# basilevh/occlusions-4d

Hardware: AMD Instinct MI355X
Metric: 4D query-points/sec (encode+decode) at n_points=14336 (higher is better)
Workload: dtype f32; 1 GPU; GREATER inference (BASELINE configs[1]): n_points=14336 video_len=12 num_sample=524288 (-> 534528 grid queries) implicit_batch_size=32768 (decoded in mini-batches of 32256 = 3584 workgroups of 9 queries; every query is decoded, results do not depend on the split), seeded random-init weights; abstract_points=531, outputs_per_query=5, parallelism=single GPU, schedule=sequential, rccl_ranks=1, decode_streams=2, decode_chunk=32256

## Files before the change

occlusions-4d_amd/csrc/common.hpp:

```cpp
#pragma once
#include <hip/hip_runtime.h>
#include <stdint.h>
#include <stdio.h>

#include "contract.hpp"

namespace occ4d {

inline int check_launch(const char* what) {
  hipError_t e = hipGetLastError();
  if (e != hipSuccess) {
    set_error("%s: %s", what, hipGetErrorString(e));
    return OCC4D_ELAUNCH;
  }
  return OCC4D_OK;
}

inline int cdiv(int64_t a, int64_t b) { return (int)((a + b - 1) / b); }

template <class Args>
int check_trunk_args(const Args& a, const char* who, int width) {
  OCC4D_REQUIRE(a.x && a.y && a.w0p && a.b0, "%s: null pointer", who);
  OCC4D_REQUIRE(a.n >= 0, "%s: n = %d", who, a.n);
  OCC4D_REQUIRE(a.ldx >= width && a.ldx % 4 == 0 && a.ldy % 4 == 0 && ((uintptr_t)a.x % 16) == 0 &&
// ... 14 lines not shown
                n_out, stage);
  const bool res_ok = a.ldr % 4 == 0 && ((uintptr_t)a.res % 16) == 0 && a.ldr >= n_out;
  if (skip) {
    OCC4D_REQUIRE(a.res && res_ok, "%s: skip rows must be 16-byte aligned with lds %% 4 == 0 and lds >= n_out", who);
  } else {
    OCC4D_REQUIRE(!a.res || res_ok, "%s: residual rows must be 16-byte aligned with ldr %% 4 == 0", who);
  }
  OCC4D_REQUIRE(!masked || (a.mask && a.ldm % 4 == 0 && ((uintptr_t)a.mask % 16) == 0 && a.ldm >= n_out),
                "%s: mask rows must be 16-byte aligned with ldm %% 4 == 0 and ldm >= n_out", who);
  return OCC4D_OK;
}

constexpr int FPS_BUCKET_MIN_POINTS = 1536;
int fps_bucket_launch(const float* xyz, int64_t stride, int n, int m, int start, int32_t* out_sorted,
                      int32_t* out_order, hipStream_t stream);


bool wgrad16_plan(int M, int N, int K, int* splits, int* m_per_split);
int wgrad16_launch(const float* g, int64_t ldg, const float* x, int64_t ldx, int M, int N, int K, int splits,
                   int m_per_split, float* part, float* part_b, int relu_x, hipStream_t stream);

int zero_rows(float* dst, int64_t ld, int64_t n, int d, hipStream_t st);
int copy_rows(float* dst, int64_t ldd, const float* src, int64_t lds, int64_t n, int d, hipStream_t st);

int cu_count();

bool f16w_enabled();
bool f16_resblock_enabled();

int pack_rowlin_f16x3_prescaled(const float* w, int64_t ldw, int n_out, float prescale, float* packed, hipStream_t st);
int rowlin_f16x3_prescaled(const float* x, int64_t ldx, float* y, int64_t ldy, const float* w_packed, const float* b,
                           int n_out, float prescale, int relu_in, const float* res, int64_t ldr, int n, hipStream_t st);

int attn16p_skew();

}
```

occlusions-4d_amd/csrc/path.hip:

```cpp
#include <algorithm>
#include <stdio.h>
#include <stdlib.h>

#include "common.hpp"

namespace {

using occ4d::cdiv;

#define TRY(expr)                  \
  do {                             \
    const int rc_ = (expr);        \
    if (rc_ != OCC4D_OK) return rc_; \
  } while (0)

constexpr int TRUNK = 416;
constexpr int ROW_CHUNK = 32768;
inline int row_step(int n) {
  static const bool balance = [] { const char* e = getenv("OCC4D_ROW_BALANCE"); return !e || e[0] != '0'; }();
  const int passes = (n + ROW_CHUNK - 1) / ROW_CHUNK;
  return passes <= 1 || !balance ? ROW_CHUNK : ((n + passes - 1) / passes + 8) / 9 * 9;
}
constexpr int64_t ALIGN = 64;

// ... 323 lines not shown
      snprintf(what, sizeof(what), "%s, merged query projection W1 Wq", who);
      TRY(check_f16_stream(prep + L.wq_x6, split_packed_floats(true, 2 * D), flag, what, "packed stream", st));
      snprintf(what, sizeof(what), "%s, layer3 weight", who);
      TRY(check_f16_stream(prep + L.w3_x6, split_packed_floats(true, w.d_out), flag, what, "packed stream", st));
    }
    if (L.bf16x6) {
      snprintf(what, sizeof(what), "%s, attention weights (attn_mlp[2] W2, merged Wp = W1 P2, pos_mlp[2] P2)", who);
      TRY(check_f16_stream(prep + L.stream6, L.f16w ? occ4d_pt_cross_attn_f16w_stream_floats()
                                                    : occ4d_pt_cross_attn_f16x3_stream_floats(), flag, what, "packed stream", st));
    }
  }
  return OCC4D_OK;
}

struct SceneTables { int64_t kt, vt, vtc, total; };
SceneTables scene_layout(const occ4d_pt_layer_weights& w, int m) {
  SceneTables s{};
  s.kt = 0;
  s.vt = up((int64_t)m * 2 * w.dim);
  s.vtc = s.vt + up((int64_t)m * w.dim);
  s.total = s.vtc + up((int64_t)m * w.dim);
  return s;
}
int layer_scene(const occ4d_pt_layer_weights& w, const LayerLayout& L, const float* prep, const float* x2, int64_t ldx2,
                int m, float* scene, hipStream_t st) {
  const SceneTables s = scene_layout(w, m);
  const int D = L.D, D2 = L.D2;
  TRY(lin(x2, ldx2, prep + L.wk, D2, nullptr, scene + s.kt, 2 * D, m, D2, 2 * D, 0, 0, nullptr, 0, st));
  TRY(lin(x2, ldx2, w.to_v, D2, nullptr, scene + s.vt, D, m, D2, D, 0, 0, nullptr, 0, st));
  TRY(lin(x2, ldx2, w.to_v, D2, w.pos2_b, scene + s.vtc, D, m, D2, D, 0, 0, nullptr, 0, st));
  return OCC4D_OK;
}

int rowlin_any(bool trunk4, const float* x, int64_t ldx, float* y, int64_t ldy, const float* wpk, const float* b, int n_out,
               int relu_in, const float* res, int64_t ldr, int n, const Events& E, hipStream_t st) {
  E.before(OCC4D_PROFILE_ROWLIN);
  const int rc = trunk4
      ? occ4d_rowlin4_f32(x, ldx, y, ldy, wpk, b, n_out, relu_in, res, ldr, nullptr, nullptr, 0, nullptr, nullptr, 0, n, st)
      : occ4d_rowlin_f32(x, ldx, y, ldy, wpk, b, n_out, relu_in, res, ldr, nullptr, nullptr, 0, nullptr, nullptr, 0, n, st);
  E.after(OCC4D_PROFILE_ROWLIN);
  return rc;
}

int rowlin_x6(bool f16, const float* x, int64_t ldx, float* y, int64_t ldy, const float* wpk, const float* b, int n_out,
              int relu_in, const float* res, int64_t ldr, int n, const Events& E, hipStream_t st, float prescale = 1.f) {
  E.before(OCC4D_PROFILE_ROWLIN);
  const int rc = split_rowlin(f16, x, ldx, y, ldy, wpk, b, n_out, relu_in, res, ldr, n, st, prescale);
  E.after(OCC4D_PROFILE_ROWLIN);
  return rc;
}

int layer_forward(const occ4d_pt_layer_weights& w, const LayerLayout& L, const float* prep, const float* x, int64_t ldx,
                  const float* pos, int64_t ps, int n, const float* x2, int64_t ldx2, const float* pos2, int64_t p2s, int m,
                  int k, const int32_t* knn_idx, const float* scene, float* out, int64_t ldo, Bump& ws,
                  const Events& E, hipStream_t st, bool dry, float* logits_out = nullptr, float* a_out = nullptr,
                  float* pe_out = nullptr) {
  const int D = L.D, h = L.h;
  const int64_t mark = ws.mark();
  const float *kt, *vt, *vtc, *aq_all = nullptr, *yfeat = x;
  int64_t ld_y = ldx;
  if (!w.cross) {
    if (w.pre_w) {
      float* y = ws.take((int64_t)n * D);
      if (!dry) TRY(lin(x, ldx, w.pre_w, w.d_in, w.pre_b, y, D, n, w.d_in, D, 0, 0, nullptr, 0, st));
      yfeat = y; ld_y = D;
    }
    float* ktb = ws.take((int64_t)n * 2 * D);
    float* vtb = ws.take((int64_t)n * D);
    float* vcb = (L.fused16p || L.bf16x6) ? ws.take((int64_t)n * D) : nullptr;
    float* aqb = ws.take((int64_t)n * 2 * D);
    if (!dry) {
      TRY(lin(yfeat, ld_y, prep + L.wk, D, nullptr, ktb, 2 * D, n, D, 2 * D, 0, 0, nullptr, 0, st));
      TRY(lin(yfeat, ld_y, w.to_v, D, nullptr, vtb, D, n, D, D, 0, 0, nullptr, 0, st));
      if (vcb) TRY(lin(yfeat, ld_y, w.to_v, D, w.pos2_b, vcb, D, n, D, D, 0, 0, nullptr, 0, st));
      TRY(lin(yfeat, ld_y, prep + L.wq, D, prep + L.bq, aqb, 2 * D, n, D, 2 * D, 0, 0, nullptr, 0, st));
    }
    kt = ktb; vt = vtb; vtc = vcb; aq_all = aqb;
    pos2 = pos; p2s = ps; m = n;
  } else if (scene) {
    const SceneTables s = scene_layout(w, m);
    kt = scene + s.kt; vt = scene + s.vt; vtc = scene + s.vtc;
  } else {
    const SceneTables s = scene_layout(w, m);
    float* tb = ws.take(s.total);
    if (!dry) TRY(layer_scene(w, L, prep, x2, ldx2, m, tb, st));
    kt = tb + s.kt; vt = tb + s.vt; vtc = tb + s.vtc;
  }
  float* agg = out;
  int64_t ld_agg = ldo;
// ... 68 lines not shown
          rc = occ4d_pt_cross_attn_f32(aq, 2 * D, qp, ps, pos2, p2s, idx, kt, 2 * D, vt, D, w.pos0_w, w.pos0_b, prep + L.wp,
                                       w.attn2_w, w.attn2_b, w.pos2_w, w.pos2_b, agg_c, ld_agg, c, m, k, D, divisor, st);
        E.after(OCC4D_PROFILE_CROSS_ATTN);
        TRY(rc);
      }
    } else if (L.fused_self16 && k == 16) {
      if (!dry)
        TRY(occ4d_pt_self_attn16_f32(aq, 2 * D, qp, ps, pos2, p2s, idx, kt, 2 * D, vt, D, w.pos0_w, w.pos0_b, prep + L.wp,
                                     w.attn2_w, w.pos2_w, w.pos2_b, agg_c, ld_agg, c, m, k, D, divisor, st));
    } else {
      const int64_t rows = (int64_t)c * k;
      float* r = ws.take(rows * h);
      float* hid = ws.take(rows * 2 * D);
      float* logits = ws.take(rows * D);
      float* pe = ws.take(rows * D);
      if (!dry) {
        TRY(occ4d_pt_pos_hidden_f32(qp, ps, pos2, p2s, idx, c, k, w.pos0_w, w.pos0_b, h, r, st));
        occ4d_linear_args a{};
        a.x = r; a.ldx = h; a.w = prep + L.wp; a.ldw = h; a.y = hid; a.ldy = 2 * D;
        a.M = (int)rows; a.K = h; a.N = 2 * D; a.relu_out = 1;
        a.add_rows = aq; a.ld_add = 2 * D; a.add_div = k; a.sub_rows = kt; a.ld_sub = 2 * D; a.sub_idx = idx;
        TRY(occ4d_linear_f32(&a, st));
        TRY(lin(hid, 2 * D, w.attn2_w, 2 * D, w.attn2_b, logits, D, (int)rows, 2 * D, D, 0, 0, nullptr, 0, st));
        TRY(lin(r, h, w.pos2_w, h, w.pos2_b, pe, D, (int)rows, h, D, 0, 0, nullptr, 0, st));
        TRY(occ4d_pt_softmax_agg_f32(logits, vt, D, pe, idx, c, k, D, divisor, agg_c, ld_agg, st));
      }
    }
    ws.release(cmark);
  }
  if (w.post_w && !dry) {
    if (L.x6rows)
      TRY(rowlin_x6(L.f16, agg, D, out, ldo, prep + L.w3_x6, w.post_b, w.d_out, 0, x, ldx, n, E, st));
    else if (L.w3_rows)
      TRY(rowlin_any(L.trunk4, agg, D, out, ldo, prep + L.w3_packed, w.post_b, w.d_out, 0, x, ldx, n, E, st));
    else
      TRY(lin(agg, D, w.post_w, D, w.post_b, out, ldo, n, D, w.d_out, 0, 0, x, ldx, st));
  }
  ws.release(mark);
  return OCC4D_OK;
}

struct DecoderLayout {
  int H, P, P4, dg, E, nB, nC;
  bool trunk, trunk4, resblock;
  bool x6trunk;
  bool f16;
  bool f16block;
  int64_t w0p[OCC4D_MAX_BLOCKS], w1p[OCC4D_MAX_BLOCKS];
  int64_t w0x[OCC4D_MAX_BLOCKS], w1x[OCC4D_MAX_BLOCKS];
  int64_t cross[OCC4D_MAX_CROSS];
  LayerLayout cl[OCC4D_MAX_CROSS];
  int64_t total;
};

int check_decoder(const occ4d_decoder_weights* w, const char* who) {
  OCC4D_REQUIRE(w, "%s: null weights", who);
  OCC4D_REQUIRE(w->n_blocks >= 1 && w->n_blocks <= OCC4D_MAX_BLOCKS && w->n_cross >= 0 && w->n_cross <= OCC4D_MAX_CROSS,
                "%s: n_blocks = %d (1 .. %d), n_cross = %d (0 .. %d)", who, w->n_blocks, OCC4D_MAX_BLOCKS, w->n_cross,
                OCC4D_MAX_CROSS);
  OCC4D_REQUIRE(w->d_hidden % 4 == 0 && w->d_hidden >= 4 && w->d_out >= 1 && w->d_in >= 3 && w->n_freq >= 0,
                "%s: d_hidden = %d must be a multiple of 4, d_in = %d >= 3 (x, y, z first)", who, w->d_hidden, w->d_in);
  const int P = w->d_in * (2 * w->n_freq + 1);
  OCC4D_REQUIRE(w->lin_in_ld >= P && w->lin_in_ld % 4 == 0, "%s: lin_in_ld = %d must be a multiple of 4 >= %d (zero-pad "
                "lin_in.weight's rows)", who, w->lin_in_ld, P);
  OCC4D_REQUIRE(w->d_latent_local >= 4 && w->d_latent_local % 4 == 0 && w->d_latent >= w->d_latent_local &&
                    (w->d_latent - w->d_latent_local) % 4 == 0,
                "%s: d_latent = %d, d_latent_local = %d (both parts multiples of 4; local_mode 'feature' / 'attention')",
// ... 84 lines not shown
    const int64_t mark = ws.mark();
    const float* q = queries + (int64_t)lo * qs;
    float* x = penult ? penult + (int64_t)lo * ld_pen : ws.take((int64_t)c * H);
    const int64_t ldx = penult ? ld_pen : H;
    int32_t* idx8 = reinterpret_cast<int32_t*>(ws.take((int64_t)c * w.k_local));
    float* w8 = ws.take((int64_t)c * w.k_local);
    int32_t* idx_att = L.nC ? reinterpret_cast<int32_t*>(ws.take((int64_t)c * w.k_cross)) : nullptr;
    float* pe = ws.take((int64_t)c * L.P4);
    float* hbuf = (L.resblock && (!L.x6trunk || L.f16block)) ? nullptr : ws.take((int64_t)c * H);
    if (!dry) {
      if (knn_local) {
        TRY(clamp_indices(knn_local + (int64_t)lo * w.k_local, (int64_t)c * w.k_local, m, idx8, st));
        TRY(occ4d_knn_dists_f32(q, qs, c, xyz, 3, m, idx8, w.k_local, 1, w8, st));
      } else {
        TRY(occ4d_knn_f32(q, qs, c, xyz, 3, m, w.k_local, 1, idx8, 0, w8, st));
      }
      TRY(occ4d_interp_weights_f32(w8, c, w.k_local, w8, st));
      if (L.nC && knn_cross) TRY(clamp_indices(knn_cross + (int64_t)lo * w.k_cross, (int64_t)c * w.k_cross, m, idx_att, st));
      else if (L.nC) TRY(occ4d_knn_f32(q, qs, c, xyz, 3, m, w.k_cross, 0, idx_att, 0, nullptr, st));
      const float* emb = q;
      int64_t ld_emb = qs;
      if (w.n_freq > 0) {
        if (L.P4 != L.P) TRY(occ4d::zero_rows(pe, L.P4, c, L.P4, st));
        TRY(occ4d_posenc_f32(q, qs, c, w.d_in, w.n_freq, (double)w.base_frequency, pe, L.P4, st));
        emb = pe; ld_emb = L.P4;
      } else {
        TRY(occ4d::zero_rows(pe, L.P4, c, L.P4, st));
        TRY(occ4d::copy_rows(pe, L.P4, q, qs, c, w.d_in, st));
        emb = pe; ld_emb = L.P4;
      }
      TRY(lin(emb, ld_emb, w.lin_in_w, w.lin_in_ld, w.lin_in_b, x, ldx, c, L.P4, H, 0, 0, nullptr, 0, st));
    }
    int next_cross = 0;
    for (int i = 0; i < L.nB; ++i) {
      if (!dry) {
        const bool fuse_ok = (flags & OCC4D_PATH_FUSED_INTERP) && L.resblock && !L.trunk4;
        const bool cross_behind = next_cross < L.nC && w.cross_after[next_cross] == i;
        const bool cross_before = i > 0 && next_cross > 0 && w.cross_after[next_cross - 1] == i - 1;
        const bool had_it = fuse_ok && i > 0 && !cross_before;
        const bool give_next = fuse_ok && i + 1 < L.nB && !cross_behind;
        if (!had_it)
          TRY(occ4d_interp_add_f32(x, ldx, scene + S.zconst + (int64_t)i * H, scene + S.ztab + (int64_t)i * H,
                                   (int64_t)L.nB * H, idx8, w8, c, w.k_local, H, st));
        if (L.f16block) {
          E.before(OCC4D_PROFILE_RESBLOCK);
          const int rc = occ4d_resblock_f16x3_f32(x, ldx, x, ldx, prep + L.w0x[i], w.fc0_b[i], w.fc1_b[i], c, st);
          E.after(OCC4D_PROFILE_RESBLOCK);
          TRY(rc);
        } else if (L.x6trunk) {
          E.before(OCC4D_PROFILE_RESBLOCK);
          int rc = split_rowlin(L.f16, x, ldx, hbuf, H, prep + L.w0x[i], w.fc0_b[i], H, 1, nullptr, 0, c, st);
          if (!rc) rc = split_rowlin(L.f16, hbuf, H, x, ldx, prep + L.w1x[i], w.fc1_b[i], H, 1, x, ldx, c, st);
          E.after(OCC4D_PROFILE_RESBLOCK);
          TRY(rc);
        } else if (L.resblock) {
          E.before(OCC4D_PROFILE_RESBLOCK);
          const float* zc = give_next ? scene + S.zconst + (int64_t)(i + 1) * H : nullptr;
          const float* zt = give_next ? scene + S.ztab + (int64_t)(i + 1) * H : nullptr;
          const int rc = L.trunk4
              ? occ4d_resblock4_f32(x, ldx, x, ldx, prep + L.w0p[i], w.fc0_b[i], prep + L.w1p[i], w.fc1_b[i], nullptr,
                                    nullptr, 0, nullptr, nullptr, 0, c, st)
              : occ4d_resblock_f32(x, ldx, x, ldx, prep + L.w0p[i], w.fc0_b[i], prep + L.w1p[i], w.fc1_b[i], zc, zt,
                                   (int64_t)L.nB * H, give_next ? idx8 : nullptr, give_next ? w8 : nullptr,
                                   give_next ? w.k_local : 0, c, st);
          E.after(OCC4D_PROFILE_RESBLOCK);
          TRY(rc);
        } else {
          TRY(lin(x, ldx, w.fc0_w[i], H, w.fc0_b[i], hbuf, H, c, H, H, act, 0, nullptr, 0, st));
          TRY(lin(hbuf, H, w.fc1_w[i], H, w.fc1_b[i], x, ldx, c, H, H, act, 0, x, ldx, st));
        }
      }
      if (next_cross < L.nC && w.cross_after[next_cross] == i) {
        const int j = next_cross++;
        TRY(layer_forward(w.cross[j], L.cl[j], prep ? prep + L.cross[j] : nullptr, x, ldx, q, qs, c, nullptr, 0, xyz, 3, m,
                          w.k_cross, idx_att, scene ? scene + S.layer[j] : nullptr, x, ldx, ws, E, st, dry));
      }
    }
    if (!dry)
      TRY(lin(x, ldx, w.lin_out_w, H, w.lin_out_b, out + (int64_t)lo * ld_out, ld_out, c, H, w.d_out, act, 0, nullptr, 0, st));
    ws.release(mark);
  }
  (void)flags;
  return OCC4D_OK;
}

}

namespace occ4d {
bool f16_resblock_enabled() {
  static const bool v = [] {
    const char* e = getenv("OCC4D_F16_RESBLOCK");
    return !e || atoi(e) != 0;
  }();
  return v;
}
bool f16w_enabled() {
  static const bool v = [] {
    const char* e = getenv("OCC4D_F16W");
    return e && atoi(e) != 0;
  }();
  return v;
}
int attn16p_skew() {
  static const int v = [] {
    const char* e = getenv("OCC4D_CA16P_SKEW");
    return e ? atoi(e) : 6;
  }();
  return v;
}
}

extern "C" int occ4d_pack_trunk_rows_f32(const float* w, int64_t ldw, int n_out, float* packed, void* stream) {
  OCC4D_REQUIRE(w && packed && n_out >= 32 && n_out % 32 == 0 && ldw >= TRUNK,
                "occ4d_pack_trunk_rows_f32: (%d, %d) weight with n_out %% 32 == 0 expected", n_out, TRUNK);
  const int64_t total = occ4d_trunk_packed_floats(n_out);
  pack_trunk_rows_kernel<<<cdiv(total, 256), 256, 0, (hipStream_t)stream>>>(w, ldw, n_out / 32, packed);
  return occ4d::check_launch("occ4d_pack_trunk_rows_f32");
}
extern "C" int occ4d_pack_trunk_cols_f32(const float* w, int64_t ldw, float* packed, void* stream) {
  OCC4D_REQUIRE(w && packed && ldw >= TRUNK, "occ4d_pack_trunk_cols_f32: (416, 416) weight expected");
  pack_trunk_cols_kernel<<<cdiv((int64_t)14 * 13312, 256), 256, 0, (hipStream_t)stream>>>(w, ldw, packed);
  return occ4d::check_launch("occ4d_pack_trunk_cols_f32");
}
extern "C" int occ4d_pack_trunk4_rows_f32(const float* w, int64_t ldw, int n_out, float* packed, void* stream) {
  OCC4D_REQUIRE(w && packed && n_out >= 16 && n_out % 16 == 0 && ldw >= TRUNK,
// ... 234 lines not shown
```

occlusions-4d_amd/csrc/trunk.hip:

```cpp
#include "tile.hpp"

namespace {

constexpr int TH = 416;
constexpr int TKG = TH / 16;
constexpr int TNS = TH / 32;
constexpr int FRAG_FLOATS = 256;
constexpr int STAGE_FRAGS = 2 * TKG;
constexpr int STAGE_FLOATS = STAGE_FRAGS * FRAG_FLOATS;
constexpr int TROWS = 128;

struct TrunkArgs {
  const float* x; int64_t ldx;
  float* y; int64_t ldy;
  const float* w0p; const float* b0;
  const float* w1p; const float* b1;
  const float* res; int64_t ldr;
  const float* zconst; const float* ztab; int64_t ldz; const int32_t* zidx; const float* zw; int kz;
  int n;
  int n_stages;
  int relu_in;
  const float* mask; int64_t ldm;
};

__device__ __forceinline__ void dma_stage(const float* __restrict__ src, const float* dst, int wave, int lane) {
#pragma unroll
  for (int i = 0; i < 7; ++i) {
    const int c = wave + 8 * i;
    if (c < STAGE_FRAGS) dma_frag(src + c * FRAG_FLOATS, lds_addr(dst) + (unsigned)c * (FRAG_FLOATS * 4), (unsigned)lane * 16u);
  }
}

__device__ __forceinline__ void dma_part(const float* __restrict__ src, const float* dst, int wave, int lane, int i) {
  const int c = wave + 8 * i;
  if (c < STAGE_FRAGS) dma_frag(src + c * FRAG_FLOATS, lds_addr(dst) + (unsigned)c * (FRAG_FLOATS * 4), (unsigned)lane * 16u);
}

__device__ __forceinline__ void interp_into(const TrunkArgs& a, int rowc, int g, f32x4* out) {
#pragma unroll
  for (int t = 0; t < TKG; ++t) {
    const f32x4 c = *reinterpret_cast<const f32x4*>(a.zconst + 16 * t + 4 * g);
    out[t].x += c.x; out[t].y += c.y; out[t].z += c.z; out[t].w += c.w;
  }
  for (int j = 0; j < a.kz; ++j) {
    const float w = a.zw[(int64_t)rowc * a.kz + j];
    const float* zr = a.ztab + (int64_t)a.zidx[(int64_t)rowc * a.kz + j] * a.ldz + 4 * g;
#pragma unroll
    for (int t = 0; t < TKG; ++t) {
      const f32x4 z = *reinterpret_cast<const f32x4*>(zr + 16 * t);
      out[t].x = fmaf(w, z.x, out[t].x); out[t].y = fmaf(w, z.y, out[t].y);
      out[t].z = fmaf(w, z.z, out[t].z); out[t].w = fmaf(w, z.w, out[t].w);
    }
  }
}

__global__ __launch_bounds__(512, 2) void resblock_kernel(const TrunkArgs a) {
  __shared__ __attribute__((aligned(16))) float bufA[STAGE_FLOATS];
  __shared__ __attribute__((aligned(16))) float bufB[STAGE_FLOATS];
  __shared__ __attribute__((aligned(16))) float s_b0[TH];
  const int tid = threadIdx.x, lane = tid & 63, wave = __builtin_amdgcn_readfirstlane(tid >> 6);
  const int r = lane & 15, g = lane >> 4;
  const int row = blockIdx.x * TROWS + wave * 16 + r;
  const int rowc = min(row, a.n - 1);

  dma_stage(a.w0p, bufA, wave, lane);
  if (tid < TH) s_b0[tid] = a.b0[tid];
  f32x4 xr[TKG], yacc[TKG];
  {
    const float* xp = a.x + (int64_t)rowc * a.ldx + 4 * g;
#pragma unroll
    for (int t = 0; t < TKG; ++t) {
#ifdef OCC4D_TR_NOPRO
      const f32x4 v = {(float)t, (float)g, (float)r, 1.f};
#else
      const f32x4 v = *reinterpret_cast<const f32x4*>(xp + 16 * t);
#endif
      const f32x4 b = *reinterpret_cast<const f32x4*>(a.b1 + 16 * t + 4 * g);
      xr[t] = relu4(v);
      yacc[t].x = v.x + b.x; yacc[t].y = v.y + b.y; yacc[t].z = v.z + b.z; yacc[t].w = v.w + b.w;
    }
  }
  dma_wait();
  __syncthreads();
  const float* const fa = bufA + lane * 4;
  const float* const fb = bufB + lane * 4;

#ifdef OCC4D_TR_STAMP
  unsigned long long tacc[4] = {0, 0, 0, 0};
  unsigned long long tprev = __builtin_amdgcn_s_memtime();
  const unsigned long long tstart = tprev;
#define STAMP(i) { const unsigned long long tn = __builtin_amdgcn_s_memtime(); tacc[i] += tn - tprev; tprev = tn; }
#else
#define STAMP(i)
#endif
  asm volatile("; OCC4D_MARK loop");
#pragma clang loop unroll(disable)
  for (int j = 0; j < TNS; ++j) {
    f32x4 h0 = *reinterpret_cast<const f32x4*>(s_b0 + 32 * j + 4 * g);
    f32x4 h1 = *reinterpret_cast<const f32x4*>(s_b0 + 32 * j + 16 + 4 * g);
    {
      f32x4 wa = *reinterpret_cast<const f32x4*>(fa);
      f32x4 wb = *reinterpret_cast<const f32x4*>(fa + TKG * FRAG_FLOATS);
#pragma unroll
      for (int t = 0; t < TKG; ++t) {
#ifndef OCC4D_TR_NODMA
        if (t >= 2 && t <= 20 && (t - 2) % 3 == 0) dma_part(a.w1p + (int64_t)j * STAGE_FLOATS, bufB, wave, lane, (t - 2) / 3);
#endif
        const f32x4 ca = wa, cb = wb;
        if (t + 1 < TKG) {
          wa = *reinterpret_cast<const f32x4*>(fa + (t + 1) * FRAG_FLOATS);
          wb = *reinterpret_cast<const f32x4*>(fa + (TKG + t + 1) * FRAG_FLOATS);
        }
        __builtin_amdgcn_sched_barrier(0);
        mfma16x2_b(ca, cb, xr[t], h0, h1);
// ... 12 lines not shown
      f32x4 wa = *reinterpret_cast<const f32x4*>(fb);
      f32x4 wb = *reinterpret_cast<const f32x4*>(fb + 2 * FRAG_FLOATS);
#pragma unroll
      for (int q = 0; q < TKG; ++q) {
        const int p = q >> 1, tt = q & 1;
#ifndef OCC4D_TR_NODMA
        if (q >= 2 && q <= 20 && (q - 2) % 3 == 0) dma_part(a.w0p + (int64_t)(j + 1) * STAGE_FLOATS, bufA, wave, lane, (q - 2) / 3);
#endif
        const f32x4 ca = wa, cb = wb;
        if (q + 1 < TKG) {
          const int pn = (q + 1) >> 1, tn = (q + 1) & 1;
          wa = *reinterpret_cast<const f32x4*>(fb + (4 * pn + tn) * FRAG_FLOATS);
          wb = *reinterpret_cast<const f32x4*>(fb + (4 * pn + 2 + tn) * FRAG_FLOATS);
        }
        __builtin_amdgcn_sched_barrier(0);
        mfma16x2_b(ca, cb, tt ? h1 : h0, yacc[2 * p], yacc[2 * p + 1]);
        __builtin_amdgcn_sched_barrier(0);
      }
    }
    STAMP(2)
#ifndef OCC4D_TR_NOBAR
    dma_wait();
    __syncthreads();
#endif
    STAMP(3)
  }
  asm volatile("; OCC4D_MARK epilogue");
#ifdef OCC4D_TR_STAMP
  if (lane == 0 && a.zw) {
    unsigned long long* o = (unsigned long long*)a.zw + (size_t)(blockIdx.x * 8 + wave) * 6;
    o[0] = tacc[0]; o[1] = tacc[1]; o[2] = tacc[2]; o[3] = tacc[3]; o[4] = tprev - tstart; o[5] = tstart;
  }
#endif
  if (a.ztab) interp_into(a, rowc, g, yacc);
#ifdef OCC4D_TR_NOEPI
  {
    float tsum = 0.f;
#pragma unroll
    for (int t = 0; t < TKG; ++t) tsum += yacc[t].x + yacc[t].y + yacc[t].z + yacc[t].w;
    if (tsum == 123.456f) a.y[0] = tsum;
    return;
  }
#endif
  if (row < a.n) {
    float* yp = a.y + (int64_t)row * a.ldy + 4 * g;
#pragma unroll
    for (int t = 0; t < TKG; ++t) *reinterpret_cast<f32x4*>(yp + 16 * t) = yacc[t];
  }
}

__device__ __forceinline__ void rowlin_stage(const TrunkArgs& a, int s, const float* __restrict__ frag, const f32x4* xr,
                                             int row, int rowc, int g, const float* next_src, const float* next_dst,
                                             int wave, int lane) {
  const int c0 = 32 * s + 4 * g;
  const f32x4 bz0 = *reinterpret_cast<const f32x4*>(a.b0 + c0);
  const f32x4 bz1 = *reinterpret_cast<const f32x4*>(a.b0 + c0 + 16);
  f32x4 o0 = {0.f, 0.f, 0.f, 0.f}, o1 = {0.f, 0.f, 0.f, 0.f};
  f32x4 r0 = {0.f, 0.f, 0.f, 0.f}, r1 = {0.f, 0.f, 0.f, 0.f};
  if (a.res) {
    r0 = *reinterpret_cast<const f32x4*>(a.res + (int64_t)rowc * a.ldr + c0);
    r1 = *reinterpret_cast<const f32x4*>(a.res + (int64_t)rowc * a.ldr + c0 + 16);
  }
  {
    f32x4 wa = *reinterpret_cast<const f32x4*>(frag);
    f32x4 wb = *reinterpret_cast<const f32x4*>(frag + TKG * FRAG_FLOATS);
#pragma unroll
    for (int t = 0; t < TKG; ++t) {
      if (t >= 2 && t <= 20 && (t - 2) % 3 == 0) dma_part(next_src, next_dst, wave, lane, (t - 2) / 3);
      const f32x4 ca = wa, cb = wb;
      if (t + 1 < TKG) {
        wa = *reinterpret_cast<const f32x4*>(frag + (t + 1) * FRAG_FLOATS);
        wb = *reinterpret_cast<const f32x4*>(frag + (TKG + t + 1) * FRAG_FLOATS);
      }
      __builtin_amdgcn_sched_barrier(0);
      mfma16x2_b(ca, cb, xr[t], o0, o1);
      __builtin_amdgcn_sched_barrier(0);
    }
  }
  o0.x += bz0.x + r0.x; o0.y += bz0.y + r0.y; o0.z += bz0.z + r0.z; o0.w += bz0.w + r0.w;
  o1.x += bz1.x + r1.x; o1.y += bz1.y + r1.y; o1.z += bz1.z + r1.z; o1.w += bz1.w + r1.w;
  if (a.ztab) {
    const f32x4 ca = *reinterpret_cast<const f32x4*>(a.zconst + c0);
    const f32x4 cb = *reinterpret_cast<const f32x4*>(a.zconst + c0 + 16);
    o0.x += ca.x; o0.y += ca.y; o0.z += ca.z; o0.w += ca.w;
    o1.x += cb.x; o1.y += cb.y; o1.z += cb.z; o1.w += cb.w;
    for (int j = 0; j < a.kz; ++j) {
      const float w = a.zw[(int64_t)rowc * a.kz + j];
      const float* zr = a.ztab + (int64_t)a.zidx[(int64_t)rowc * a.kz + j] * a.ldz + c0;
      const f32x4 za = *reinterpret_cast<const f32x4*>(zr);
      const f32x4 zb = *reinterpret_cast<const f32x4*>(zr + 16);
      o0.x = fmaf(w, za.x, o0.x); o0.y = fmaf(w, za.y, o0.y); o0.z = fmaf(w, za.z, o0.z); o0.w = fmaf(w, za.w, o0.w);
      o1.x = fmaf(w, zb.x, o1.x); o1.y = fmaf(w, zb.y, o1.y); o1.z = fmaf(w, zb.z, o1.z); o1.w = fmaf(w, zb.w, o1.w);
    }
  }
  if (a.mask) {
    const f32x4 m0 = *reinterpret_cast<const f32x4*>(a.mask + (int64_t)rowc * a.ldm + c0);
    const f32x4 m1 = *reinterpret_cast<const f32x4*>(a.mask + (int64_t)rowc * a.ldm + c0 + 16);
    o0.x = m0.x > 0.f ? o0.x : 0.f; o0.y = m0.y > 0.f ? o0.y : 0.f; o0.z = m0.z > 0.f ? o0.z : 0.f; o0.w = m0.w > 0.f ? o0.w : 0.f;
    o1.x = m1.x > 0.f ? o1.x : 0.f; o1.y = m1.y > 0.f ? o1.y : 0.f; o1.z = m1.z > 0.f ? o1.z : 0.f; o1.w = m1.w > 0.f ? o1.w : 0.f;
  }
  if (row < a.n) {
    float* yp = a.y + (int64_t)row * a.ldy + c0;
    *reinterpret_cast<f32x4*>(yp) = o0;
    *reinterpret_cast<f32x4*>(yp + 16) = o1;
  }
}

__global__ __launch_bounds__(512, 2) void rowlin_kernel(const TrunkArgs a) {
  __shared__ __attribute__((aligned(16))) float bufA[STAGE_FLOATS];
  __shared__ __attribute__((aligned(16))) float bufB[STAGE_FLOATS];
  const int tid = threadIdx.x, lane = tid & 63, wave = __builtin_amdgcn_readfirstlane(tid >> 6);
  const int r = lane & 15, g = lane >> 4;
  const int row = blockIdx.x * TROWS + wave * 16 + r;
  const int rowc = min(row, a.n - 1);
  dma_stage(a.w0p, bufA, wave, lane);
  f32x4 xr[TKG];
  {
    const float* xp = a.x + (int64_t)rowc * a.ldx + 4 * g;
#pragma unroll
    for (int t = 0; t < TKG; ++t) {
      const f32x4 v = *reinterpret_cast<const f32x4*>(xp + 16 * t);
      xr[t] = a.relu_in ? relu4(v) : v;
    }
  }
  dma_wait();
  __syncthreads();
#pragma clang loop unroll(disable)
  for (int s = 0; s < a.n_stages; s += 2) {
    rowlin_stage(a, s, bufA + lane * 4, xr, row, rowc, g, a.w0p + (int64_t)(s + 1) * STAGE_FLOATS, bufB, wave, lane);
    dma_wait();
    __syncthreads();
    if (s + 1 < a.n_stages)
      rowlin_stage(a, s + 1, bufB + lane * 4, xr, row, rowc, g, a.w0p + (int64_t)(s + 2) * STAGE_FLOATS, bufA, wave, lane);
    dma_wait();
    __syncthreads();
  }
}

int rowlin_launch(const char* who, const float* x, int64_t ldx, float* y, int64_t ldy, const float* w_packed, const float* b,
                  int n_out, int relu_in, const float* res, int64_t ldr, const float* zconst, const float* ztab, int64_t ldz,
                  const int32_t* zidx, const float* zw, int kz, bool masked, const float* mask, int64_t ldm, int n,
                  void* stream) {
  if (n == 0) return OCC4D_OK;
  TrunkArgs a{x, ldx, y, ldy, w_packed, b, nullptr, nullptr, res, ldr, zconst, ztab, ldz, zidx, zw, kz, n,
              n_out / 32, relu_in, mask, ldm};
  if (int rc = occ4d::check_rowlin_args(a, who, TH, 32, n_out, masked)) return rc;
  rowlin_kernel<<<occ4d::cdiv(n, TROWS), 512, 0, (hipStream_t)stream>>>(a);
  return occ4d::check_launch(who);
}

}

extern "C" int occ4d_trunk_width(void) { return TH; }
extern "C" int64_t occ4d_trunk_packed_floats(int n_out) { return (int64_t)(n_out / 32 + 1) * STAGE_FLOATS; }

extern "C" int occ4d_resblock_f32(const float* x, int64_t ldx, float* y, int64_t ldy, const float* w0_packed,
                                  const float* b0, const float* w1_packed, const float* b1, const float* zconst,
                                  const float* ztab, int64_t ldz, const int32_t* zidx, const float* zw, int kz, int n,
                                  void* stream) {
  TrunkArgs a{x, ldx, y, ldy, w0_packed, b0, w1_packed, b1, nullptr, 0, zconst, ztab, ldz, zidx, zw, kz, n, TNS, 1, nullptr, 0};
  if (n == 0) return OCC4D_OK;
  if (int rc = occ4d::check_trunk_args(a, "occ4d_resblock_f32", TH)) return rc;
  OCC4D_REQUIRE(w1_packed && b1 && ((uintptr_t)w1_packed % 16) == 0 && ((uintptr_t)b1 % 16) == 0 && ldy >= TH,
                "occ4d_resblock_f32: second layer weights / bias missing or misaligned");
  resblock_kernel<<<occ4d::cdiv(n, TROWS), 512, 0, (hipStream_t)stream>>>(a);
  return occ4d::check_launch("occ4d_resblock_f32");
// ... 17 lines not shown
```

Baseline: 4.529 million query-points/s.

## Stage deduplicated interpolation rows in LDS and fuse interp into cross-layer rowlin

Each 128-row workgroup deduplicates its kNN indices into a small LDS row table using a bitmap, prefix sums and slot indices. The distinct z-table rows are staged into shared memory, reusing the freed stage buffers in resblock and a double-buffered slice image in rowlin. Interpolation then gathers from LDS instead of scattered global loads, and falls back to direct gathers when a tile has more than 64 distinct rows. Separately, the path fuses the next block's interpolation term into the cross-attention output rowlin, removing a standalone interp_add launch. The costs are extra LDS and barriers, which may reduce occupancy, plus the dedupe overhead.

```diff
diff --git a/occlusions-4d_amd/csrc/common.hpp b/occlusions-4d_amd/csrc/common.hpp
--- a/occlusions-4d_amd/csrc/common.hpp
+++ b/occlusions-4d_amd/csrc/common.hpp
@@ -70,6 +70,8 @@
 int rowlin_f16x3_prescaled(const float* x, int64_t ldx, float* y, int64_t ldy, const float* w_packed, const float* b,
                            int n_out, float prescale, int relu_in, const float* res, int64_t ldr, int n, hipStream_t st);
 
+bool staged_interp_enabled();
+
 int attn16p_skew();
 
 }
diff --git a/occlusions-4d_amd/csrc/path.hip b/occlusions-4d_amd/csrc/path.hip
--- a/occlusions-4d_amd/csrc/path.hip
+++ b/occlusions-4d_amd/csrc/path.hip
@@ -379,12 +379,15 @@
   return OCC4D_OK;
 }
 
+struct ZTerm { const float* zconst; const float* ztab; int64_t ldz; const int32_t* idx; const float* w; int k; };
+
 int rowlin_any(bool trunk4, const float* x, int64_t ldx, float* y, int64_t ldy, const float* wpk, const float* b, int n_out,
-               int relu_in, const float* res, int64_t ldr, int n, const Events& E, hipStream_t st) {
+               int relu_in, const float* res, int64_t ldr, int n, const Events& E, hipStream_t st, const ZTerm* z = nullptr) {
   E.before(OCC4D_PROFILE_ROWLIN);
   const int rc = trunk4
       ? occ4d_rowlin4_f32(x, ldx, y, ldy, wpk, b, n_out, relu_in, res, ldr, nullptr, nullptr, 0, nullptr, nullptr, 0, n, st)
-      : occ4d_rowlin_f32(x, ldx, y, ldy, wpk, b, n_out, relu_in, res, ldr, nullptr, nullptr, 0, nullptr, nullptr, 0, n, st);
+      : z ? occ4d_rowlin_f32(x, ldx, y, ldy, wpk, b, n_out, relu_in, res, ldr, z->zconst, z->ztab, z->ldz, z->idx, z->w, z->k, n, st)
+          : occ4d_rowlin_f32(x, ldx, y, ldy, wpk, b, n_out, relu_in, res, ldr, nullptr, nullptr, 0, nullptr, nullptr, 0, n, st);
   E.after(OCC4D_PROFILE_ROWLIN);
   return rc;
 }
@@ -401,7 +404,7 @@
                   const float* pos, int64_t ps, int n, const float* x2, int64_t ldx2, const float* pos2, int64_t p2s, int m,
                   int k, const int32_t* knn_idx, const float* scene, float* out, int64_t ldo, Bump& ws,
                   const Events& E, hipStream_t st, bool dry, float* logits_out = nullptr, float* a_out = nullptr,
-                  float* pe_out = nullptr) {
+                  float* pe_out = nullptr, const ZTerm* zterm = nullptr) {
   const int D = L.D, h = L.h;
   const int64_t mark = ws.mark();
   const float *kt, *vt, *vtc, *aq_all = nullptr, *yfeat = x;
@@ -536,7 +539,7 @@
     if (L.x6rows)
       TRY(rowlin_x6(L.f16, agg, D, out, ldo, prep + L.w3_x6, w.post_b, w.d_out, 0, x, ldx, n, E, st));
     else if (L.w3_rows)
-      TRY(rowlin_any(L.trunk4, agg, D, out, ldo, prep + L.w3_packed, w.post_b, w.d_out, 0, x, ldx, n, E, st));
+      TRY(rowlin_any(L.trunk4, agg, D, out, ldo, prep + L.w3_packed, w.post_b, w.d_out, 0, x, ldx, n, E, st, zterm));
     else
       TRY(lin(agg, D, w.post_w, D, w.post_b, out, ldo, n, D, w.d_out, 0, 0, x, ldx, st));
   }
@@ -687,13 +690,15 @@
       TRY(lin(emb, ld_emb, w.lin_in_w, w.lin_in_ld, w.lin_in_b, x, ldx, c, L.P4, H, 0, 0, nullptr, 0, st));
     }
     int next_cross = 0;
+    const bool fuse_cross = L.resblock && !L.trunk4 && !L.x6trunk && occ4d::staged_interp_enabled();
+    const bool fuse_ok = fuse_cross || ((flags & OCC4D_PATH_FUSED_INTERP) && L.resblock && !L.trunk4 && !L.x6trunk);
+    bool had_it = false;
     for (int i = 0; i < L.nB; ++i) {
+      const bool cross_behind = next_cross < L.nC && w.cross_after[next_cross] == i;
+      const bool give_next = fuse_ok && i + 1 < L.nB && !cross_behind;
+      const bool cross_gives = !dry && fuse_cross && i + 1 < L.nB && cross_behind && L.cl[next_cross].w3_rows &&
+                               !L.cl[next_cross].x6rows && !L.cl[next_cross].trunk4 && w.cross[next_cross].d_out == H;
       if (!dry) {
-        const bool fuse_ok = (flags & OCC4D_PATH_FUSED_INTERP) && L.resblock && !L.trunk4;
-        const bool cross_behind = next_cross < L.nC && w.cross_after[next_cross] == i;
-        const bool cross_before = i > 0 && next_cross > 0 && w.cross_after[next_cross - 1] == i - 1;
-        const bool had_it = fuse_ok && i > 0 && !cross_before;
-        const bool give_next = fuse_ok && i + 1 < L.nB && !cross_behind;
         if (!had_it)
           TRY(occ4d_interp_add_f32(x, ldx, scene + S.zconst + (int64_t)i * H, scene + S.ztab + (int64_t)i * H,
                                    (int64_t)L.nB * H, idx8, w8, c, w.k_local, H, st));
@@ -725,11 +730,17 @@
           TRY(lin(hbuf, H, w.fc1_w[i], H, w.fc1_b[i], x, ldx, c, H, H, act, 0, x, ldx, st));
         }
       }
-      if (next_cross < L.nC && w.cross_after[next_cross] == i) {
+      if (cross_behind) {
         const int j = next_cross++;
+        ZTerm zt{};
+        if (cross_gives)
+          zt = ZTerm{scene + S.zconst + (int64_t)(i + 1) * H, scene + S.ztab + (int64_t)(i + 1) * H, (int64_t)L.nB * H, idx8, w8,
+                     w.k_local};
         TRY(layer_forward(w.cross[j], L.cl[j], prep ? prep + L.cross[j] : nullptr, x, ldx, q, qs, c, nullptr, 0, xyz, 3, m,
-                          w.k_cross, idx_att, scene ? scene + S.layer[j] : nullptr, x, ldx, ws, E, st, dry));
+                          w.k_cross, idx_att, scene ? scene + S.layer[j] : nullptr, x, ldx, ws, E, st, dry, nullptr, nullptr,
+                          nullptr, cross_gives ? &zt : nullptr));
       }
+      had_it = give_next || cross_gives;
     }
     if (!dry)
       TRY(lin(x, ldx, w.lin_out_w, H, w.lin_out_b, out + (int64_t)lo * ld_out, ld_out, c, H, w.d_out, act, 0, nullptr, 0, st));
@@ -746,6 +757,13 @@
   static const bool v = [] {
     const char* e = getenv("OCC4D_F16_RESBLOCK");
     return !e || atoi(e) != 0;
+  }();
+  return v;
+}
+bool staged_interp_enabled() {
+  static const bool v = [] {
+    const char* e = getenv("OCC4D_STAGED_INTERP");
+    return !e || e[0] != '0';
   }();
   return v;
 }
diff --git a/occlusions-4d_amd/csrc/rowstage.hpp b/occlusions-4d_amd/csrc/rowstage.hpp
--- /dev/null
+++ b/occlusions-4d_amd/csrc/rowstage.hpp
@@ -0,0 +1,61 @@
+#pragma once
+#include "common.hpp"
+
+namespace {
+
+constexpr int RS_THREADS = 512;
+constexpr int RS_ROWS = 128;
+constexpr int RS_KMAX = 16;
+constexpr int RS_BITS = 32 * RS_THREADS;
+constexpr int RS_CAP = 64;
+
+struct RowStage {
+  unsigned char slot[RS_ROWS * RS_KMAX];
+  unsigned bm[RS_THREADS];
+  unsigned short pre[RS_THREADS];
+  int rows[RS_CAP];
+  unsigned wsum[RS_THREADS / 64];
+  int bad;
+};
+
+__device__ __forceinline__ int rs_dedupe(RowStage& rs, const int32_t* __restrict__ idx, int nrefs, int tid) {
+  const int lane = tid & 63, wave = tid >> 6;
+  rs.bm[tid] = 0u;
+  if (tid == 0) rs.bad = 0;
+  __syncthreads();
+  for (int e = tid; e < nrefs; e += RS_THREADS) {
+    const int j = idx[e];
+    if ((unsigned)j < (unsigned)RS_BITS) atomicOr(&rs.bm[j >> 5], 1u << (j & 31));
+    else rs.bad = 1;
+  }
+  __syncthreads();
+  const unsigned mine = rs.bm[tid];
+  const unsigned cnt = (unsigned)__builtin_popcount(mine);
+  unsigned inc = cnt;
+#pragma unroll
+  for (int o = 1; o < 64; o <<= 1) {
+    const unsigned v = (unsigned)__shfl_up((int)inc, o, 64);
+    if (lane >= o) inc += v;
+  }
+  if (lane == 63) rs.wsum[wave] = inc;
+  __syncthreads();
+  unsigned below = 0, total = 0;
+#pragma unroll
+  for (int w = 0; w < RS_THREADS / 64; ++w) {
+    const unsigned s = rs.wsum[w];
+    if (w < wave) below += s;
+    total += s;
+  }
+  if (rs.bad || total > (unsigned)RS_CAP) return -1;
+  unsigned at = below + inc - cnt;
+  rs.pre[tid] = (unsigned short)at;
+  for (unsigned b = mine; b; b &= b - 1) rs.rows[at++] = 32 * tid + (__builtin_ffs((int)b) - 1);
+  __syncthreads();
+  for (int e = tid; e < nrefs; e += RS_THREADS) {
+    const int j = idx[e];
+    rs.slot[e] = (unsigned char)(rs.pre[j >> 5] + __builtin_popcount(rs.bm[j >> 5] & ((1u << (j & 31)) - 1u)));
+  }
+  return (int)total;
+}
+
+}
diff --git a/occlusions-4d_amd/csrc/trunk.hip b/occlusions-4d_amd/csrc/trunk.hip
--- a/occlusions-4d_amd/csrc/trunk.hip
+++ b/occlusions-4d_amd/csrc/trunk.hip
@@ -1,4 +1,5 @@
 #include "tile.hpp"
+#include "rowstage.hpp"
 
 namespace {
 
@@ -9,6 +10,7 @@
 constexpr int STAGE_FRAGS = 2 * TKG;
 constexpr int STAGE_FLOATS = STAGE_FRAGS * FRAG_FLOATS;
 constexpr int TROWS = 128;
+static_assert(TROWS == RS_ROWS && RS_CAP * TH <= 2 * STAGE_FLOATS, "the staged interpolation term lives in the two stage buffers");
 
 struct TrunkArgs {
   const float* x; int64_t ldx;
@@ -36,28 +38,72 @@
   if (c < STAGE_FRAGS) dma_frag(src + c * FRAG_FLOATS, lds_addr(dst) + (unsigned)c * (FRAG_FLOATS * 4), (unsigned)lane * 16u);
 }
 
-__device__ __forceinline__ void interp_into(const TrunkArgs& a, int rowc, int g, f32x4* out) {
-#pragma unroll
-  for (int t = 0; t < TKG; ++t) {
-    const f32x4 c = *reinterpret_cast<const f32x4*>(a.zconst + 16 * t + 4 * g);
-    out[t].x += c.x; out[t].y += c.y; out[t].z += c.z; out[t].w += c.w;
-  }
-  for (int j = 0; j < a.kz; ++j) {
-    const float w = a.zw[(int64_t)rowc * a.kz + j];
-    const float* zr = a.ztab + (int64_t)a.zidx[(int64_t)rowc * a.kz + j] * a.ldz + 4 * g;
-#pragma unroll
-    for (int t = 0; t < TKG; ++t) {
-      const f32x4 z = *reinterpret_cast<const f32x4*>(zr + 16 * t);
-      out[t].x = fmaf(w, z.x, out[t].x); out[t].y = fmaf(w, z.y, out[t].y);
-      out[t].z = fmaf(w, z.z, out[t].z); out[t].w = fmaf(w, z.w, out[t].w);
-    }
-  }
+__device__ __forceinline__ float* zslot_base(float* bufA, float* bufB, int slot) {
+  return (slot < RS_CAP / 2 ? bufA : bufB) + (slot & (RS_CAP / 2 - 1)) * TH;
+}
+
+__device__ __forceinline__ void zstage_rows(const TrunkArgs& a, const RowStage& rs, int nrows, float* bufA, float* bufB, int tid) {
+  constexpr int C4 = TH / 4, PER = (RS_CAP * C4 + RS_THREADS - 1) / RS_THREADS;
+  f32x4 v[PER];
+#pragma unroll
+  for (int i = 0; i < PER; ++i) {
+    const int e = tid + RS_THREADS * i, slot = e / C4, c = e - slot * C4;
+    if (slot < nrows) v[i] = *reinterpret_cast<const f32x4*>(a.ztab + (int64_t)rs.rows[slot] * a.ldz + 4 * c);
+  }
+#pragma unroll
+  for (int i = 0; i < PER; ++i) {
+    const int e = tid + RS_THREADS * i, slot = e / C4, c = e - slot * C4;
+    if (slot < nrows) *reinterpret_cast<f32x4*>(zslot_base(bufA, bufB, slot) + 4 * (c ^ ((slot >> 1) & 7))) = v[i];
+  }
+}
+
+template <bool STAGED>
+__device__ __forceinline__ void interp_into(const TrunkArgs& a, const RowStage& rs, float* bufA, float* bufB, int rowc, int lrow,
+                                            int g, f32x4* out) {
+  constexpr int HALF = TKG / 2;
+#pragma unroll
+  for (int half = 0; half < 2; ++half) {
+    f32x4 s[HALF];
+#pragma unroll
+    for (int u = 0; u < HALF; ++u) s[u] = f32x4{0.f, 0.f, 0.f, 0.f};
+    for (int j = 0; j < a.kz; ++j) {
+      const float w = a.zw[(int64_t)rowc * a.kz + j];
+      const float *pe, *po;
+      if (STAGED) {
+        const int slot = rs.slot[lrow * a.kz + j], sw = (slot >> 1) & 7, hi = sw >> 2;
+        const float* p = zslot_base(bufA, bufB, slot) + 4 * (g ^ (sw & 3));
+        pe = p + 16 * hi; po = p - 16 * hi;
+      } else {
+        pe = po = a.ztab + (int64_t)a.zidx[(int64_t)rowc * a.kz + j] * a.ldz + 4 * g;
+      }
+#pragma unroll
+      for (int u = 0; u < HALF; ++u) {
+        const int t = HALF * half + u;
+        const f32x4 z = *reinterpret_cast<const f32x4*>(((t & 1) ? po : pe) + 16 * t);
+        s[u].x += w * z.x; s[u].y += w * z.y; s[u].z += w * z.z; s[u].w += w * z.w;
+      }
+    }
+#pragma unroll
+    for (int u = 0; u < HALF; ++u) {
+      const int t = HALF * half + u;
+      const f32x4 c = *reinterpret_cast<const f32x4*>(a.zconst + 16 * t + 4 * g);
+      s[u].x += c.x; s[u].y += c.y; s[u].z += c.z; s[u].w += c.w;
+      out[t].x += s[u].x; out[t].y += s[u].y; out[t].z += s[u].z; out[t].w += s[u].w;
+    }
+  }
+}
+
+__device__ __forceinline__ int zdedupe(const TrunkArgs& a, RowStage& rs, int tid) {
+  if (!a.ztab || a.kz > RS_KMAX) return -1;
+  const int row0 = blockIdx.x * TROWS;
+  return __builtin_amdgcn_readfirstlane(rs_dedupe(rs, a.zidx + (int64_t)row0 * a.kz, min(TROWS, a.n - row0) * a.kz, tid));
 }
 
 __global__ __launch_bounds__(512, 2) void resblock_kernel(const TrunkArgs a) {
   __shared__ __attribute__((aligned(16))) float bufA[STAGE_FLOATS];
   __shared__ __attribute__((aligned(16))) float bufB[STAGE_FLOATS];
   __shared__ __attribute__((aligned(16))) float s_b0[TH];
+  __shared__ RowStage rs;
   const int tid = threadIdx.x, lane = tid & 63, wave = __builtin_amdgcn_readfirstlane(tid >> 6);
   const int r = lane & 15, g = lane >> 4;
   const int row = blockIdx.x * TROWS + wave * 16 + r;
@@ -80,6 +126,7 @@
       yacc[t].x = v.x + b.x; yacc[t].y = v.y + b.y; yacc[t].z = v.z + b.z; yacc[t].w = v.w + b.w;
     }
   }
+  const int zrows = zdedupe(a, rs, tid);
   dma_wait();
   __syncthreads();
   const float* const fa = bufA + lane * 4;
@@ -158,7 +205,15 @@
     o[0] = tacc[0]; o[1] = tacc[1]; o[2] = tacc[2]; o[3] = tacc[3]; o[4] = tprev - tstart; o[5] = tstart;
   }
 #endif
-  if (a.ztab) interp_into(a, rowc, g, yacc);
+  if (a.ztab) {
+    if (zrows >= 0) {
+      zstage_rows(a, rs, zrows, bufA, bufB, tid);
+      __syncthreads();
+      interp_into<true>(a, rs, bufA, bufB, rowc, rowc - blockIdx.x * TROWS, g, yacc);
+    } else {
+      interp_into<false>(a, rs, bufA, bufB, rowc, 0, g, yacc);
+    }
+  }
 #ifdef OCC4D_TR_NOEPI
   {
     float tsum = 0.f;
@@ -175,10 +230,29 @@
   }
 }
 
+constexpr int ZS_LD = 36;
+constexpr int ZS_FLOATS = RS_CAP * ZS_LD;
+struct ZSlices {
+  const RowStage* rs;
+  int rows;
+  int lrow;
+};
+__device__ __forceinline__ f32x4 zslice_load(const TrunkArgs& a, const ZSlices& z, int s, int tid) {
+  f32x4 v = {0.f, 0.f, 0.f, 0.f};
+  if ((tid >> 3) < z.rows) v = *reinterpret_cast<const f32x4*>(a.ztab + (int64_t)z.rs->rows[tid >> 3] * a.ldz + 32 * s + 4 * (tid & 7));
+  return v;
+}
+__device__ __forceinline__ void zslice_store(const ZSlices& z, float* img, int tid, f32x4 v) {
+  if ((tid >> 3) < z.rows) *reinterpret_cast<f32x4*>(img + (tid >> 3) * ZS_LD + 4 * (tid & 7)) = v;
+}
+
 __device__ __forceinline__ void rowlin_stage(const TrunkArgs& a, int s, const float* __restrict__ frag, const f32x4* xr,
                                              int row, int rowc, int g, const float* next_src, const float* next_dst,
-                                             int wave, int lane) {
+                                             int wave, int lane, const ZSlices& zs, const float* zcur, float* znxt) {
   const int c0 = 32 * s + 4 * g;
+  const bool znext = zs.rows >= 0 && s + 1 < a.n_stages;
+  f32x4 zv = {0.f, 0.f, 0.f, 0.f};
+  if (znext) zv = zslice_load(a, zs, s + 1, 64 * wave + lane);
   const f32x4 bz0 = *reinterpret_cast<const f32x4*>(a.b0 + c0);
   const f32x4 bz1 = *reinterpret_cast<const f32x4*>(a.b0 + c0 + 16);
   f32x4 o0 = {0.f, 0.f, 0.f, 0.f}, o1 = {0.f, 0.f, 0.f, 0.f};
@@ -206,19 +280,34 @@
   o0.x += bz0.x + r0.x; o0.y += bz0.y + r0.y; o0.z += bz0.z + r0.z; o0.w += bz0.w + r0.w;
   o1.x += bz1.x + r1.x; o1.y += bz1.y + r1.y; o1.z += bz1.z + r1.z; o1.w += bz1.w + r1.w;
   if (a.ztab) {
+    f32x4 s0 = {0.f, 0.f, 0.f, 0.f}, s1 = {0.f, 0.f, 0.f, 0.f};
+    if (zs.rows >= 0) {
+      for (int j = 0; j < a.kz; ++j) {
+        const float w = a.zw[(int64_t)rowc * a.kz + j];
+        const float* zr = zcur + (int)zs.rs->slot[zs.lrow * a.kz + j] * ZS_LD + 4 * g;
+        const f32x4 za = *reinterpret_cast<const f32x4*>(zr);
+        const f32x4 zb = *reinterpret_cast<const f32x4*>(zr + 16);
+        s0.x += w * za.x; s0.y += w * za.y; s0.z += w * za.z; s0.w += w * za.w;
+        s1.x += w * zb.x; s1.y += w * zb.y; s1.z += w * zb.z; s1.w += w * zb.w;
+      }
+    } else {
+      for (int j = 0; j < a.kz; ++j) {
+        const float w = a.zw[(int64_t)rowc * a.kz + j];
+        const float* zr = a.ztab + (int64_t)a.zidx[(int64_t)rowc * a.kz + j] * a.ldz + c0;
+        const f32x4 za = *reinterpret_cast<const f32x4*>(zr);
+        const f32x4 zb = *reinterpret_cast<const f32x4*>(zr + 16);
+        s0.x += w * za.x; s0.y += w * za.y; s0.z += w * za.z; s0.w += w * za.w;
+        s1.x += w * zb.x; s1.y += w * zb.y; s1.z += w * zb.z; s1.w += w * zb.w;
+      }
+    }
     const f32x4 ca = *reinterpret_cast<const f32x4*>(a.zconst + c0);
     const f32x4 cb = *reinterpret_cast<const f32x4*>(a.zconst + c0 + 16);
-    o0.x += ca.x; o0.y += ca.y; o0.z += ca.z; o0.w += ca.w;
-    o1.x += cb.x; o1.y += cb.y; o1.z += cb.z; o1.w += cb.w;
-    for (int j = 0; j < a.kz; ++j) {
-      const float w = a.zw[(int64_t)rowc * a.kz + j];
-      const float* zr = a.ztab + (int64_t)a.zidx[(int64_t)rowc * a.kz + j] * a.ldz + c0;
-      const f32x4 za = *reinterpret_cast<const f32x4*>(zr);
-      const f32x4 zb = *reinterpret_cast<const f32x4*>(zr + 16);
-      o0.x = fmaf(w, za.x, o0.x); o0.y = fmaf(w, za.y, o0.y); o0.z = fmaf(w, za.z, o0.z); o0.w = fmaf(w, za.w, o0.w);
-      o1.x = fmaf(w, zb.x, o1.x); o1.y = fmaf(w, zb.y, o1.y); o1.z = fmaf(w, zb.z, o1.z); o1.w = fmaf(w, zb.w, o1.w);
-    }
-  }
+    s0.x += ca.x; s0.y += ca.y; s0.z += ca.z; s0.w += ca.w;
+    s1.x += cb.x; s1.y += cb.y; s1.z += cb.z; s1.w += cb.w;
+    o0.x += s0.x; o0.y += s0.y; o0.z += s0.z; o0.w += s0.w;
+    o1.x += s1.x; o1.y += s1.y; o1.z += s1.z; o1.w += s1.w;
+  }
+  if (znext) zslice_store(zs, znxt, 64 * wave + lane, zv);
   if (a.mask) {
     const f32x4 m0 = *reinterpret_cast<const f32x4*>(a.mask + (int64_t)rowc * a.ldm + c0);
     const f32x4 m1 = *reinterpret_cast<const f32x4*>(a.mask + (int64_t)rowc * a.ldm + c0 + 16);
@@ -235,6 +324,9 @@
 __global__ __launch_bounds__(512, 2) void rowlin_kernel(const TrunkArgs a) {
   __shared__ __attribute__((aligned(16))) float bufA[STAGE_FLOATS];
   __shared__ __attribute__((aligned(16))) float bufB[STAGE_FLOATS];
+  __shared__ __attribute__((aligned(16))) float zimg0[ZS_FLOATS];
+  __shared__ __attribute__((aligned(16))) float zimg1[ZS_FLOATS];
+  __shared__ RowStage rs;
   const int tid = threadIdx.x, lane = tid & 63, wave = __builtin_amdgcn_readfirstlane(tid >> 6);
   const int r = lane & 15, g = lane >> 4;
   const int row = blockIdx.x * TROWS + wave * 16 + r;
@@ -249,15 +341,17 @@
       xr[t] = a.relu_in ? relu4(v) : v;
     }
   }
+  const ZSlices zs{&rs, zdedupe(a, rs, tid), rowc - (int)blockIdx.x * TROWS};
+  if (zs.rows >= 0) zslice_store(zs, zimg0, tid, zslice_load(a, zs, 0, tid));
   dma_wait();
   __syncthreads();
 #pragma clang loop unroll(disable)
   for (int s = 0; s < a.n_stages; s += 2) {
-    rowlin_stage(a, s, bufA + lane * 4, xr, row, rowc, g, a.w0p + (int64_t)(s + 1) * STAGE_FLOATS, bufB, wave, lane);
+    rowlin_stage(a, s, bufA + lane * 4, xr, row, rowc, g, a.w0p + (int64_t)(s + 1) * STAGE_FLOATS, bufB, wave, lane, zs, zimg0, zimg1);
     dma_wait();
     __syncthreads();
     if (s + 1 < a.n_stages)
-      rowlin_stage(a, s + 1, bufB + lane * 4, xr, row, rowc, g, a.w0p + (int64_t)(s + 2) * STAGE_FLOATS, bufA, wave, lane);
+      rowlin_stage(a, s + 1, bufB + lane * 4, xr, row, rowc, g, a.w0p + (int64_t)(s + 2) * STAGE_FLOATS, bufA, wave, lane, zs, zimg1, zimg0);
     dma_wait();
     __syncthreads();
   }
diff --git a/profiles/staged_interp_hist.py b/profiles/staged_interp_hist.py
--- /dev/null
+++ b/profiles/staged_interp_hist.py
@@ -0,0 +1,43 @@
+import os
+import sys
+
+import torch
+
+ROOT = os.path.dirname(os.path.dirname(os.path.abspath(__file__)))
+sys.path.insert(0, ROOT)
+import bench
+import occlusions4d_amd as pk
+
+TILE, CAP, BITS = 128, 64, 16384
+kind = sys.argv[1] if len(sys.argv) > 1 else 'greater'
+dev = torch.device('cuda', 0)
+pa, ia, inf = pk.configs.model_args(kind, bench.N_POINTS)
+esd, _ = pk.configs.synthetic_weights(pa, ia, bench.SEED)
+enc = pk.model.PointCompletionNetV3(**pa).to(dev).eval()
+enc.load_state_dict(esd)
+pcl = pk.configs.synthetic_pcl(kind, bench.N_POINTS, bench.VIDEO_LEN, bench.SEED).to(dev)
+q = pk.geometry.sample_implicit_points_blind_device(bench.NUM_SAMPLE, inf['min_z'], inf['cube_bounds'], 3, inf['data_kind'],
+                                                    inf['cube_mode'], 'grid', dev)
+with torch.no_grad():
+    abstract = enc(pcl, False)[0].squeeze(0)
+m = abstract.shape[0]
+batch = pk.inference.decode_chunk(bench.BATCH)
+counts = []
+for k in (8, 14):
+    per_tile = []
+    for b in range(0, q.shape[0], batch):
+        rows, lo = q[b:b + batch], 0
+        for c in pk.ops.path_row_chunks(rows.shape[0]):
+            idx = pk.ops.knn(rows[lo:lo + c], abstract, k, metric=1 if k == 8 else 0).long()
+            lo += c
+            for t in range(0, c, TILE):
+                per_tile.append(int(torch.unique(idx[t:t + TILE]).numel()))
+    counts.append((k, torch.tensor(per_tile)))
+for k, c in counts:
+    hist = torch.bincount(c)
+    print('%d-NN lists, %d queries over %d abstract points, %d tiles of %d rows: distinct rows min %d mean %.1f p95 %d max %d'
+          % (k, q.shape[0], m, c.numel(), TILE, int(c.min()), float(c.double().mean()), int(c.double().quantile(0.95)), int(c.max())))
+    print('   histogram (distinct rows: tiles): ' + ' '.join('%d:%d' % (i, int(n)) for i, n in enumerate(hist.tolist()) if n))
+    if k == 8:
+        print('   capacity %d rows, bitmap %d rows (table: %d): %d of %d tiles fall back to direct gathers (%.3f %%)'
+              % (CAP, BITS, m, int((c > CAP).sum()), c.numel(), 100.0 * float((c > CAP).double().mean())))
```

Result: no change. 4.573 million query-points/s, median of 6 (+1.0%).
